# kfirc1503/generative-audio

Hardware: AMD Instinct MI355X
Metric: spectrogram-frames/sec, NPPC K=5 FullSubNet+ train step (higher is better)
Workload: dtype bf16

## Files before the change

### generative-audio_amd/csrc/train_ops.hip

```cpp
#include "common.h"
#include "nppc_hip.h"

namespace {

template <typename T>
__global__ __launch_bounds__(256) void transpose_kernel(const T* __restrict__ in, T* __restrict__ out, int rows, int cols,
                                                        long ld_in, long ld_out, long sIn, long sOut, int relu) {
  __shared__ float tile[32][33];
  in += (size_t)blockIdx.z * sIn;
  out += (size_t)blockIdx.z * sOut;
  const int r0 = blockIdx.x * 32, c0 = blockIdx.y * 32;
  const int tx = threadIdx.x & 31, ty = threadIdx.x >> 5;
  for (int i = ty; i < 32; i += 8) {
    const int r = r0 + i, c = c0 + tx;
    float v = 0.f;
    if (r < rows && c < cols) v = to_f32<T>(in[(size_t)r * ld_in + c]);
    if (relu) v = fmaxf(v, 0.f);
    tile[i][tx] = v;
  }
  __syncthreads();
  for (int i = ty; i < 32; i += 8) {
    const int c = c0 + i, r = r0 + tx;
    if (c < cols && r < rows) out[(size_t)c * ld_out + r] = from_f32<T>(tile[tx][i]);
  }
// ... 308 lines not shown
  for (long e = (long)blockIdx.x * blockDim.x + threadIdx.x; e < total; e += (long)gridDim.x * blockDim.x) {
    const int r = (int)(e / ncols), c = (int)(e % ncols);
    float s = 0.f;
    for (int k = 0; k < S; ++k) s += slabs[(size_t)k * slab_stride + (size_t)r * ld + col0 + c];
    int rr = r;
    if (permH > 0) {
      const int u = r >> 2, gp = r & 3;
      const int tg = gp == 0 ? 0 : (gp == 1 ? 2 : (gp == 2 ? 1 : 3));
      rr = tg * permH + u;
    }
    float* d = dst + (size_t)rr * dst_ld + c;
    *d = accumulate ? *d + s : s;
  }
}

__global__ void reduce_slabs_t_kernel(const float* __restrict__ slabs, int S, long slab_stride, long ld, float* __restrict__ dst,
                                      long dst_ld, int rows, int ncols, long sSlab, long sDst) {
  slabs += (size_t)blockIdx.z * sSlab;
  dst += (size_t)blockIdx.z * sDst;
  __shared__ float tile[32][33];
  const int c0 = blockIdx.x * 32, r0 = blockIdx.y * 32;
  const int tx = threadIdx.x & 31, ty = threadIdx.x >> 5;
  for (int i = ty; i < 32; i += 8) {
    const int c = c0 + i, r = r0 + tx;
    float a = 0.f;
    if (c < ncols && r < rows)
      for (int s = 0; s < S; ++s) a += slabs[(size_t)s * slab_stride + (size_t)c * ld + r];
    tile[i][tx] = a;
  }
  __syncthreads();
  for (int i = ty; i < 32; i += 8) {
    const int r = r0 + i, c = c0 + tx;
    if (r < rows && c < ncols) dst[(size_t)r * dst_ld + c] = tile[tx][i];
  }
}

__global__ void adam_kernel(float* __restrict__ p, const float* __restrict__ g, float* __restrict__ m, float* __restrict__ v,
                            long n, float lr, float b1, float b2, float eps, float wd, float bc1, float bc2_sqrt,
                            float gscale, const double* __restrict__ sumsq, float max_norm,
                            const unsigned* const* __restrict__ guards = nullptr, int n_guards = 0, float* poison = nullptr) {
  for (int i = 0; i < n_guards; ++i)
    if (*guards[i] != 0u) {
      if (poison && blockIdx.x == 0 && threadIdx.x == 0) *poison = __builtin_nanf("");
      return;
    }
  if (sumsq) {
    const float total = (float)sqrt(sumsq[0]) * gscale;
    const float coef = max_norm / (total + 1e-6f);
    gscale *= coef < 1.f ? coef : 1.f;
  }
  for (long i = (long)blockIdx.x * blockDim.x + threadIdx.x; i < n; i += (long)gridDim.x * blockDim.x) {
    float gi = g[i] * gscale;
    const float pi = p[i];
    if (wd != 0.f) gi += wd * pi;
    const float mi = b1 * m[i] + (1.f - b1) * gi;
    const float vi = b2 * v[i] + (1.f - b2) * gi * gi;
    m[i] = mi;
    v[i] = vi;
    const float denom = sqrtf(vi) / bc2_sqrt + eps;
    p[i] = pi - (lr / bc1) * (mi / denom);
  }
}

}

extern "C" {
// ... 147 lines not shown
  const double Nn = (double)F * (2 * nb + 4) * Tv;
  dim3 grid(Tv, B);
  hipStream_t s = (hipStream_t)stream;
  if (prec == NPPC_PREC_BF16)
    hipLaunchKernelGGL(sb_unfold_bwd_kernel<bf16_t>, grid, dim3(256), sm, s, (const bf16_t*)dx, scale, D, mult, (bf16_t*)dX0,
                       ldX, B, F, Tp, nb, Geff, Fo, KX, Nseq, Nn);
  else
    hipLaunchKernelGGL(sb_unfold_bwd_kernel<float>, grid, dim3(256), sm, s, (const float*)dx, scale, D, mult, (float*)dX0, ldX,
                       B, F, Tp, nb, Geff, Fo, KX, Nseq, Nn);
  NPPC_CHECK_LAUNCH();
  return NPPC_OK;
}

int nppc_reduce_slabs(const float* slabs, int S, long slab_stride, long ld, float* dst, long dst_ld, int rows, int col0,
                      int ncols, int permH, int accumulate, long sSlab, long sDst, int batch, void* stream) {
  if (!slabs || !dst || S < 1 || rows <= 0 || ncols <= 0) return NPPC_EBADARG;
  const long total = (long)rows * ncols;
  const int gx = (int)((total + 255) / 256 > 1024 ? 1024 : (total + 255) / 256);
  hipLaunchKernelGGL(reduce_slabs_kernel, dim3(gx, 1, batch), dim3(256), 0, (hipStream_t)stream, slabs, S, slab_stride, ld,
                     dst, dst_ld, rows, col0, ncols, permH, accumulate, sSlab, sDst);
  NPPC_CHECK_LAUNCH();
  return NPPC_OK;
}

int nppc_reduce_slabs_t(const float* slabs, int S, long slab_stride, long ld, float* dst, long dst_ld, int rows, int ncols,
                        long sSlab, long sDst, int batch, void* stream) {
  if (!slabs || !dst || S < 1 || rows <= 0 || ncols <= 0 || batch < 1) return NPPC_EBADARG;
  hipLaunchKernelGGL(reduce_slabs_t_kernel, dim3(ceil_div(ncols, 32), ceil_div(rows, 32), batch), dim3(256), 0,
                     (hipStream_t)stream, slabs, S, slab_stride, ld, dst, dst_ld, rows, ncols, sSlab, sDst);
  NPPC_CHECK_LAUNCH();
  return NPPC_OK;
}

int nppc_adam_step(float* p, const float* g, float* m, float* v, long n, double lr, double b1, double b2, double eps,
                   double wd, int step, double gscale, void* stream) {
  if (!p || !g || !m || !v || n <= 0 || step < 1) return NPPC_EBADARG;
  const double bc1 = 1.0 - pow(b1, (double)step);
  const double bc2s = sqrt(1.0 - pow(b2, (double)step));
  const int grid = (int)((n + 255) / 256 > 2048 ? 2048 : (n + 255) / 256);
  hipLaunchKernelGGL(adam_kernel, dim3(grid), dim3(256), 0, (hipStream_t)stream, p, g, m, v, n, (float)lr, (float)b1, (float)b2,
                     (float)eps, (float)wd, (float)bc1, (float)bc2s, (float)gscale, (const double*)nullptr, 0.f);
  NPPC_CHECK_LAUNCH();
  return NPPC_OK;
}

int nppc_adam_step_guarded(float* p, const float* g, float* m, float* v, long n, double lr, double b1, double b2, double eps,
                           double wd, int step, double gscale, const void* guards, int n_guards, float* poison, void* stream) {
  if (!p || !g || !m || !v || n <= 0 || step < 1 || n_guards < 0 || (n_guards > 0 && !guards)) return NPPC_EBADARG;
  const double bc1 = 1.0 - pow(b1, (double)step);
  const double bc2s = sqrt(1.0 - pow(b2, (double)step));
  const int grid = (int)((n + 255) / 256 > 2048 ? 2048 : (n + 255) / 256);
  hipLaunchKernelGGL(adam_kernel, dim3(grid), dim3(256), 0, (hipStream_t)stream, p, g, m, v, n, (float)lr, (float)b1, (float)b2,
                     (float)eps, (float)wd, (float)bc1, (float)bc2s, (float)gscale, (const double*)nullptr, 0.f,
                     (const unsigned* const*)guards, n_guards, poison);
  NPPC_CHECK_LAUNCH();
  return NPPC_OK;
}

int nppc_adam_step_clip(float* p, const float* g, float* m, float* v, long n, double lr, double b1, double b2, double eps,
                        double wd, int step, double gscale, const double* sumsq, double max_norm, void* stream) {
  if (!p || !g || !m || !v || !sumsq || n <= 0 || step < 1 || !(max_norm > 0)) return NPPC_EBADARG;
  const double bc1 = 1.0 - pow(b1, (double)step);
  const double bc2s = sqrt(1.0 - pow(b2, (double)step));
  const int grid = (int)((n + 255) / 256 > 2048 ? 2048 : (n + 255) / 256);
  hipLaunchKernelGGL(adam_kernel, dim3(grid), dim3(256), 0, (hipStream_t)stream, p, g, m, v, n, (float)lr, (float)b1, (float)b2,
                     (float)eps, (float)wd, (float)bc1, (float)bc2s, (float)gscale, sumsq, (float)max_norm);
// ... 6 lines not shown
```

### generative-audio_amd/nppc_audio/_hip.py

```python
import ctypes
import os

import torch

_HERE = os.path.dirname(os.path.abspath(__file__))
LIB_PATH = os.environ.get("NPPC_HIP_LIB") or os.path.join(_HERE, "libnppc_hip.so")

PREC_BF16 = 0
PREC_F32 = 1
_ERR = {1: "bad argument", 2: "kernel launch failed", 3: "unsupported shape/configuration"}

_lib = None

c_p = ctypes.c_void_p
c_i = ctypes.c_int
c_l = ctypes.c_long
c_f = ctypes.c_float


def lib():
    global _lib
    if _lib is None:
        if not os.path.exists(LIB_PATH):
            raise RuntimeError(
# ... 108 lines not shown
                         I, I, I, I, I, F, L, L, L, I, I, P],
    "nppc_tcn_mid_bwd_finish": [P, L, P, L, I, I, I, P, P, P, P, P, P, P, P, P, P, I, I, L, L, I, I, P],
    "nppc_gemm_nt_colsum": [I, I, P, L, L, P, L, L, P, L, L, P, L, P, L, L, I, I, I, I, I, I, I, P, P],
    "nppc_gemm_nt_gn": [I, P, L, L, P, L, L, P, L, L, P, P, L, P, L, L, P, L, D, F, I, I, I, I, I, I, I, P],
    "nppc_tcn_pack_sconv": [I, P, P, P, P, P, P, P, I, I, I, I, I, I, L, L, L, L, P],
    "nppc_gemm_nt_splitk": [I, P, L, P, L, P, L, I, I, L, I, P],
    "nppc_gemm_tn_splitk": [P, L, P, L, P, L, I, I, L, I, P],
    "nppc_gemm_tn_splitk_rowsum": [P, L, P, L, P, L, I, I, L, I, P, P],
    "nppc_gemm_tn_splitk2": [P, L, P, L, I, P, L, I, P, L, I, L, I, P, P],
    "nppc_gemm_tn_splitk_batched": [P, L, L, P, L, L, P, L, L, I, I, L, I, I, P],
    "nppc_reduce_slabs_t": [P, I, L, L, P, L, I, I, L, L, I, P],
    "nppc_gemm_tn_splitk_taps": [P, L, P, L, P, L, I, I, L, I, I, I, P],
    "nppc_tcn_dwconv": [I, P, P, P, P, P, P, P, P, P, I, I, I, I, I, I, F, L, L, L, I, P],
    "nppc_tcn_gn_apply": [I, P, P, P, P, P, I, I, I, I, I, F, L, L, L, I, P],
    "nppc_pack_matrix": [I, P, P, I, I, I, I, I, P],
    "nppc_pack_matrix_batched": [I, P, P, I, I, I, I, I, I, I, L, L, L, L, P],
    "nppc_subband_mean": [I, P, I, P, I, L, P, P, P, I, I, I, I, I, P],
    "nppc_subband_stage": [I, P, I, P, I, L, P, P, I, I, I, I, I, I, I, I, P],
    "nppc_sb_head": [I, P, P, P, P, L, I, I, I, I, I, P],
    "nppc_gram": [P, P, P, P, P, I, I, L, P],
    "nppc_combine": [P, P, P, P, P, P, P, I, I, L, P],
    "nppc_gs_solve": [P, P, P, I, I, I, P],
    "nppc_gs_bwd_solve": [P, P, P, P, I, I, I, P],
    "nppc_loss_solve": [P, P, P, P, P, P, P, P, P, P, I, I, P],
    "nppc_loss_bwd_coef": [P, P, P, F, F, P, I, I, P],
    "nppc_loss_bwd_coef_dev": [P, P, P, P, F, F, P, I, I, P],
    "nppc_transpose": [I, P, P, I, I, L, L, L, L, I, I, P],
    "nppc_colsum": [I, P, P, I, I, L, L, L, I, P, L, P],
    "nppc_colsum_scratch_elems": [I, I, I, PL],
    "nppc_sb_head_bwd": [I, P, P, P, P, P, P, L, I, I, I, I, I, P],
    "nppc_subband_stage_bwd": [I, P, P, P, P, P, P, I, I, I, I, I, L, I, I, I, P],
    "nppc_subband_unfold_bwd": [I, P, P, P, P, P, I, I, I, I, I, I, I, I, P],
    "nppc_reduce_slabs": [P, I, L, L, P, L, I, I, I, I, I, L, L, I, P],
    "nppc_adam_step": [P, P, P, P, L, D, D, D, D, D, I, D, P],
    "nppc_adam_step_guarded": [P, P, P, P, L, D, D, D, D, D, I, D, P, I, P, P],
    "nppc_loss_solve_eps": [P, P, P, P, P, P, P, P, P, P, I, I, D, I, P],
    "nppc_loss_solve_obj": [P, P, P, P, P, P, P, P, P, P, I, I, D, I, F, P, P],
    "nppc_mix_snr": [P, P, P, F, P, P, P, I, I, P],
    "nppc_inpaint_prepare": [P, P, P, I, F, P, P, P, I, I, I, I, I, P],
    "nppc_time_to_spec_mask": [P, P, I, I, I, I, I, I, P],
    "nppc_stft_pair": [P, P, P, P, I, I, I, I, P],
    "nppc_dropout": [I, P, L, L, I, F, L, I, P, P],
    "nppc_pca_work_elems": [I, I, I, PL],
    "nppc_pca_batch": [P, I, I, I, I, P, P, P, P, P, P, P],
    "nppc_pair_loss": [P, P, P, P, P, P, P, P, P, I, I, L, D, P],
    "nppc_pair_loss_bwd": [P, P, P, P, F, F, P, I, I, L, P],
    "nppc_metric_rows": [P, P, P, P, P, L, P],
    "nppc_rows_gram": [P, I, P, I, L, P, P],
    "nppc_sumsq": [P, L, P, P],
    "nppc_adam_step_clip": [P, P, P, P, L, D, D, D, D, D, I, D, P, D, P],
    "nppc_logmag": [P, P, L, I, L, P, P],
    "nppc_standardize": [P, P, L, I, L, P, P, P],
    "nppc_unet_stage_map": [I, P, L, P, L, I, I, I, I, P],
    "nppc_conv_pack": [I, P, P, P, I, I, I, I, I, I, I, P],
    "nppc_conv_fwd": [I, P, L, P, P, L, P, P, P, F, I, I, I, I, I, I, I, P],
    "nppc_conv_fwd_stats": [I, P, L, P, P, L, P, I, I, I, I, I, I, I, P, P],
    "nppc_bn_stats_from_parts": [P, I, I, I, I, I, P, P, P],
    "nppc_conv_wgrad": [I, P, L, P, L, P, I, I, I, I, I, I, I, P],
    "nppc_conv_thin_part_elems": [PL],
    "nppc_conv3x3_thin_fwd": [I, P, L, P, P, P, P, F, P, L, I, I, I, I, I, P],
    "nppc_conv3x3_thin_wgrad": [I, P, L, P, L, P, P, I, I, I, I, I, P],
    "nppc_conv1x1_thin_fwd": [I, P, L, P, P, P, L, I, I, I, I, I, P],
    "nppc_conv1x1_thin_bwd_data": [I, P, L, P, P, L, I, I, I, I, I, P],
    "nppc_conv1x1_thin_wgrad": [I, P, L, P, L, P, P, I, I, I, I, I, P],
    "nppc_conv_wgrad_transposed": [I, I],
    "nppc_conv_wgrad_reduce": [I, P, I, I, I, P, I, I, I, P],
# ... 74 lines not shown
    "nppc_flac_decode_host": [P, L, P, L, P, L, P],
    "nppc_flac_work_elems": [L, PL],
    "nppc_flac_scan": [P, L, P, I, P, L, P],
    "nppc_flac_parse": [P, P, I, P, L, P],
    "nppc_flac_chain": [P, P, I, P, L, P, P],
    "nppc_flac_decode": [P, P, I, P, L, P, L, P, L, P],
    "nppc_flac_stream_md5": [P, L, P, P, P],
    "nppc_flac_md5_host": [P, L, I, I, P],
    "nppc_flac_md5": [P, L, P, I, P, P, P, P, P, P],
    "nppc_resample_sinc_shape": [I, I, I, I, I, PI, PL, PL, PL, PI],
    "nppc_resample_sinc": [P, L, P, I, P, I, I, I, I, I, P, L, P],
}
_bound = set()
PROFILE = None


def call(name, *args):
    fn = getattr(lib(), name)
    if name not in _bound:
        fn.argtypes = SIGS[name]
        fn.restype = c_i
        _bound.add(name)
    conv = [ptr(a) if (isinstance(a, torch.Tensor) or a is None) else a for a in args]
    if PROFILE is None:
        check(fn(*conv), name)
        return
    e0, e1 = torch.cuda.Event(enable_timing=True), torch.cuda.Event(enable_timing=True)
    e0.record()
    check(fn(*conv), name)
    e1.record()
    PROFILE.append((name, e0, e1))


def colsum(prec, M, out, rows, cols, ld, sM, sOut, batch, scratch_for, s):
    n = ctypes.c_long()
    call("nppc_colsum_scratch_elems", rows, cols, batch, ctypes.byref(n))
    sc = scratch_for(n.value)
    call("nppc_colsum", prec, M, out, rows, cols, ld, sM, sOut, batch, sc, sc.numel(), s)
```

### generative-audio_amd/nppc_audio/engine.py

```python
import ctypes
import os

import numpy as np
import torch

from . import _hip as H
from .ops_lstm import (PackedLSTM, PackedLSTMBwd, ROW_PAD, WGRAD_SPLITS, bwd_head_fusable, forward_x_ld, lstm2_backward, lstm2_forward,
                       own_workspaces, padded_rows,
                       rows_view, workspace)

TCN_HIDDEN = 512
TCN_DILATIONS = (1, 2, 5, 9, 1, 2, 5, 9)
BRANCHES = ("", "_real", "_imag")
EPI_PLAIN, EPI_PRELU_STATS, EPI_RESIDUAL, EPI_RELU, EPI_PLAIN_F32, EPI_MASK_POS = 0, 1, 2, 3, 4, 5


def rup(a, b):
    return (a + b - 1) // b * b


TCN_WGRAD_ON_SIDE = os.environ.get("NPPC_TCN_WGRAD_SIDE", "1") != "0"
TCN_WGRAD_SPLITS = int(os.environ.get("NPPC_TCN_S2", "8"))
FC_WGRAD_AT_END = os.environ.get("NPPC_FC_AT_END", "1") != "0"
TCN_WGRAD_MAIN_BLOCKS = int(os.environ.get("NPPC_TCN_WGRAD_MAIN_BLOCKS", "1"))
MID_FINISH_DEFER = os.environ.get("NPPC_MID_FINISH_DEFER", "1") != "0"
COLSUM_IN_GEMM = os.environ.get("NPPC_COLSUM_IN_GEMM", "1") != "0"
TN_PAIRED = os.environ.get("NPPC_TN_PAIRED", "1") != "0"
FUSED_HEAD = int(os.environ.get("NPPC_FUSED_HEAD", "3"))


class FlatParams:

    def __init__(self, module, device):
        named = list(module.named_parameters())
        total = sum(p.numel() for _, p in named)
        self.flat = torch.empty(total, dtype=torch.float32, device=device)
        self.grad = None
        self.off = {}
        o = 0
        for n, p in named:
            k = p.numel()
            self.flat[o:o + k].copy_(p.detach().reshape(-1))
            p.data = self.flat[o:o + k].view(p.shape)
            self.off[n] = (o, tuple(p.shape))
            o += k
        self.named = named

    def view(self, name):
        o, shp = self.off[name]
        return self.flat[o:o + int(np.prod(shp))].view(shp)

    def gview(self, name):
        o, shp = self.off[name]
        return self.grad[o:o + int(np.prod(shp))].view(shp)

    def version(self):
        return (self.flat._version, sum(p._version for _, p in self.named))

    def ensure_grad(self):
        if self.grad is None:
# ... 336 lines not shown
        q = "sb_model.sequence_model."
        Rr = Tv * Nseq
        ws = lambda name, shape, dtype=dt, zero=False: workspace(("eng", id(self), name), shape, dtype, dev, zero)
        jobs = [
            (dg1, 0, x_rows, KX, ("ih", q + "weight_ih_l0", q + "bias_ih_l0", q + "bias_hh_l0")),
            (dg2, 0, x_rows, KX, ("bias", None, q + "bias_ih_l1", q + "bias_hh_l1")),
            (dg2, 0, h1_rows, Hd, ("w", q + "weight_ih_l1")),
        ]
        if Tv > 1:
            jobs += [(dg1, Nseq, h1_rows, Hd, ("w", q + "weight_hh_l0")), (dg2, Nseq, h2_rows, Hd, ("w", q + "weight_hh_l1"))]

        def scatter(slab, S, rows, ncolsN, dest):
            kind = dest[0]
            if kind in ("ih", "w"):
                ncol = I if kind == "ih" else Hd
                H.call("nppc_reduce_slabs", slab, S, rows * ncolsN, ncolsN, self.g(dest[1]), ncol, K4, 0, ncol, Hd, 0, 0, 0, 1, s)
            if kind in ("ih", "bias"):
                H.call("nppc_reduce_slabs", slab, S, rows * ncolsN, ncolsN, self.g(dest[2]), 1, K4, I, 1, Hd, 0, 0, 0, 1, s)
                self.g(dest[3]).copy_(self.g(dest[2]))

        if self.prec == H.PREC_BF16 and K4 % 128 == 0 and Hd % 64 == 0 and KX % 64 == 0:
            S = WGRAD_SPLITS
            assert 64 * S <= ROW_PAD
            slab = ws("slab", (S * K4 * max(Hd, KX),), torch.float32)
            fold_bias = K4 % 256 == 0 and Hd % 128 == 0 and (K4 // 256) * (Hd // 128) * S >= 256
            if (guards is not None and TN_PAIRED and fold_bias and Hd % 192 == 0 and KX == 64 and Tv > 1
                    and (K4 // 256) * (Hd // 192 + 1) * S >= 256):
                h1_guard, h2_guard = guards
                rows = (Rr + 64 * S - 1) // (64 * S) * (64 * S)
                slab = ws("slab2", (S * K4 * 2 * Hd,), torch.float32)
                rsum = ws("rowsum", (S, K4), torch.float32)
                H.call("nppc_gemm_tn_splitk2", dg1, K4, h1_guard, Hd, Hd, x_rows, KX, KX, slab, Hd + KX, K4, rows, S, None, s)
                n1 = K4 * (Hd + KX)
                H.call("nppc_reduce_slabs", slab, S, n1, Hd + KX, self.g(q + "weight_hh_l0"), Hd, K4, 0, Hd, Hd, 0, 0, 0, 1, s)
                H.call("nppc_reduce_slabs", slab, S, n1, Hd + KX, self.g(q + "weight_ih_l0"), I, K4, Hd, I, Hd, 0, 0, 0, 1, s)
                H.call("nppc_reduce_slabs", slab, S, n1, Hd + KX, self.g(q + "bias_ih_l0"), 1, K4, Hd + I, 1, Hd, 0, 0, 0, 1, s)
                self.g(q + "bias_hh_l0").copy_(self.g(q + "bias_ih_l0"))
                H.call("nppc_gemm_tn_splitk2", dg2, K4, h1_rows, Hd, Hd, h2_guard, Hd, Hd, slab, 2 * Hd, K4, rows, S, rsum, s)
                n2 = K4 * 2 * Hd
                H.call("nppc_reduce_slabs", slab, S, n2, 2 * Hd, self.g(q + "weight_ih_l1"), Hd, K4, 0, Hd, Hd, 0, 0, 0, 1, s)
                H.call("nppc_reduce_slabs", slab, S, n2, 2 * Hd, self.g(q + "weight_hh_l1"), Hd, K4, Hd, Hd, Hd, 0, 0, 0, 1, s)
                H.call("nppc_reduce_slabs", rsum, S, K4, 1, self.g(q + "bias_ih_l1"), 1, K4, 0, 1, Hd, 0, 0, 0, 1, s)
                self.g(q + "bias_hh_l1").copy_(self.g(q + "bias_ih_l1"))
                jobs = []
            for dg, off, inp, width, dest in jobs:
                rows = (Rr - off + 64 * S - 1) // (64 * S) * (64 * S)
                if fold_bias and dest[0] == "bias":
                    continue
                if fold_bias and dest == ("w", q + "weight_ih_l1"):
                    rsum = ws("rowsum", (S, K4), torch.float32)
                    H.call("nppc_gemm_tn_splitk_rowsum", dg.view(-1)[off * K4:], K4, inp, width, slab, width, K4, width, rows, S,
                           rsum, s)
                    H.call("nppc_reduce_slabs", rsum, S, K4, 1, self.g(q + "bias_ih_l1"), 1, K4, 0, 1, Hd, 0, 0, 0, 1, s)
                    self.g(q + "bias_hh_l1").copy_(self.g(q + "bias_ih_l1"))
                else:
                    H.call("nppc_gemm_tn_splitk", dg.view(-1)[off * K4:], K4, inp, width, slab, width, K4, width, rows, S, s)
                scatter(slab, S, K4, width, dest)
            if head is not None:
                dyt_rows, O = head
                rows = (Rr + 64 * S - 1) // (64 * S) * (64 * S)
                H.call("nppc_gemm_tn_splitk", h2_rows, Hd, dyt_rows, 16, slab, 64, Hd, 64, rows, S, s)
                H.call("nppc_reduce_slabs_t", slab, S, Hd * 64, 64, self.g("sb_model.fc_output_layer.weight"), Hd, O, Hd, 0, 0, 1, s)
                H.colsum(self.prec, dyt_rows, self.g("sb_model.fc_output_layer.bias"), Rr, O, 16, 0, 0, 1,
                         lambda n: ws("cs_head", (n,), torch.float32), s)
            return
        bk = 64 if self.prec == H.PREC_BF16 else 32
        Sg = max(1, min(64, Rr // (16 * bk)))
        Rp = rup(Rr, bk * Sg)
        K4p, Hp, KXp = rup(K4, 128), rup(Hd, 128), rup(KX, 128)
        dgT = [ws("dg1T", (K4p, Rp), zero=True), ws("dg2T", (K4p, Rp), zero=True)]
        for src, dst in ((dg1, dgT[0]), (dg2, dgT[1])):
            H.call("nppc_transpose", self.prec, src, dst, Rr, K4, K4, Rp, 0, 0, 0, 1, s)
        slab = ws("slab", (Sg * K4p * max(Hp, KXp),), torch.float32)
        for dg, off, inp, width, dest in jobs:
            wp = rup(width, 128)
            name = f"inT_{id(inp)}_{off}"
# ... 94 lines not shown
            dXL = [ws(f"dX_{i}", (3, B, Tp, ldC)) for i in range(9)]
            a2L = [ws(f"a2_{i}", (3, B, Tp, TCN_HIDDEN), zero=True) for i in range(8)]
            h2L = [ws(f"h2b_{i}", (3, B, Tp, TCN_HIDDEN)) for i in range(8)]
            dXa, dXb = dXL[8], dXL[7]
        else:
            dXa = ws("dXa", (3, B, Tp, ldC))
            dXb = ws("dXb", (3, B, Tp, ldC))

        bk = 64 if prec == H.PREC_BF16 else 32
        cs_ok = tn_ok and COLSUM_IN_GEMM and ldF % bk == 0 and TCN_HIDDEN % bk == 0
        cp_all = ws("colpart", (8, 3, R // 128, ldC), torch.float32) if cs_ok else None
        cpL = [cp_all[i] for i in range(8)] if cs_ok else None
        if cs_ok:
            H.call("nppc_gemm_nt_colsum", prec, EPI_MASK_POS, dpre_fb, ldF, R * ldF, self.WfcT, ldF, ldC * ldF, dXa, ldC, R * ldC,
                   None, 0, X8, ldC, R * ldC, R, ldC, ldF, Tp, Tv, C, 3, cpL[7], s)
        else:
            H.call("nppc_gemm_nt", prec, EPI_MASK_POS, dpre_fb, ldF, R * ldF, self.WfcT, ldF, ldC * ldF, dXa, ldC, R * ldC, None, 0,
                   X8, ldC, R * ldC, None, 0, None, 0, R, ldC, ldF, Tp, Tv, C, 0, 3, 1, s)
        sAct = B * Tp * TCN_HIDDEN
        h1b = ws("h1b", (3, B, Tp, TCN_HIDDEN))
        h2b = ws("h2b", (3, B, Tp, TCN_HIDDEN))
        Smid = ws("Smid", (3, B, TCN_HIDDEN // 64, 8), torch.float64)
        n_part = H.mid_bwd_part_elems(B, TCN_HIDDEN, Tp, 3)
        Pmid = ws("Pmid", (8, n_part), torch.float32)
        lay = self.fp.off["fb_model.sequence_model.1.conv1x1.weight"][0] - self.fp.off["fb_model.sequence_model.0.conv1x1.weight"][0]

        def finish_mid(lo, hi):
            pre_ = f"fb_model.sequence_model.{lo}."
            H.call("nppc_tcn_mid_bwd_finish", Pmid[lo], n_part, cpL[lo] if cs_ok else None, 3 * (R // 128) * ldC, R // 128, ldC, C,
                   self.g(pre_ + "norm2.weight"), self.g(pre_ + "norm2.bias"), self.g(pre_ + "norm1.weight"), self.g(pre_ + "norm1.bias"),
                   self.g(pre_ + "depthwise_conv.weight"), self.g(pre_ + "depthwise_conv.bias"), self.g(pre_ + "prelu1.weight"),
                   self.g(pre_ + "prelu2.weight"), self.g(pre_ + "conv1x1.bias"), self.g(pre_ + "sconv.bias") if cs_ok else None,
                   B, TCN_HIDDEN, sP, lay, 3, hi - lo, s)
        early = self.grad_range_hook is not None and self.early_buckets_ok
        defer_finish = MID_FINISH_DEFER
        dXo, dXi = dXa, dXb
        for i in range(7, -1, -1):
            pre = f"fb_model.sequence_model.{i}."
            dil = TCN_DILATIONS[i]
            st1, st2 = d["stats"][i, 0], d["stats"][i, 1]
            y1, y2, Xin = d["y1"][i], d["y2"][i], d["X"][i]
            if tn_ok:
                dXo, dXi, a2, h2b = dXL[i + 1], dXL[i], a2L[i], h2L[i]
            else:
                a2 = d["a2"]
            if not cs_ok:
                H.colsum(prec, dXo, self.g(pre + "sconv.bias"), R, C, ldC, R * ldC, sP, 3,
                         lambda n: ws("cs_sconv", (n,), torch.float32), s)
            H.call("nppc_gemm_nt", prec, EPI_PLAIN, dXo, ldC, R * ldC, self.W2T[i], ldC, TCN_HIDDEN * ldC, h1b, TCN_HIDDEN,
                   sAct, None, 0, None, 0, 0, None, 0, None, 0, R, TCN_HIDDEN, ldC, Tp, Tv, TCN_HIDDEN, 0, 3, 1, s)
            H.call("nppc_tcn_mid_bwd", prec, h1b, y2, y1, st1, st2, Smid, Pmid[i], self.p(pre + "norm1.weight"), self.p(pre + "norm1.bias"),
                   self.p(pre + "norm2.weight"), self.p(pre + "norm2.bias"), self.p(pre + "depthwise_conv.weight"),
                   self.p(pre + "prelu1.weight"), self.p(pre + "prelu2.weight"), a2, h2b, self.g(pre + "norm2.weight"),
                   self.g(pre + "norm2.bias"), self.g(pre + "norm1.weight"), self.g(pre + "norm1.bias"),
                   self.g(pre + "depthwise_conv.weight"), self.g(pre + "depthwise_conv.bias"), self.g(pre + "prelu1.weight"),
                   self.g(pre + "prelu2.weight"), self.g(pre + "conv1x1.bias"),
                   cpL[i] if cs_ok else None, R // 128, ldC, C, self.g(pre + "sconv.bias") if cs_ok else None,
                   B, TCN_HIDDEN, Tp, Tv, dil, 1e-8, sAct, B * 2, sP, 3, 0 if defer_finish else 1, s)
            if i == 4 and early and defer_finish:
                finish_mid(4, 8)
            if tn_ok:
                inline = i < TCN_WGRAD_MAIN_BLOCKS
                wslab = ws("slab_main", (3 * S2 * TCN_HIDDEN * ldC,), torch.float32) if inline else slab2

                def sconv_wgrad(a2=a2, dXo=dXo, dest=self.g(pre + "sconv.weight"), wslab=wslab):
                    q = H.stream()
                    H.call("nppc_gemm_tn_splitk_batched", a2, TCN_HIDDEN, sAct, dXo, ldC, R * ldC, wslab, ldC,
                           S2 * TCN_HIDDEN * ldC, TCN_HIDDEN, ldC, R, S2, 3, q)
                    H.call("nppc_reduce_slabs_t", wslab, S2, TCN_HIDDEN * ldC, ldC, dest, TCN_HIDDEN, C, TCN_HIDDEN,
                           S2 * TCN_HIDDEN * ldC, sP, 3, q)
                if inline:
                    sconv_wgrad()
                else:
                    on_side(sconv_wgrad)
            else:
                H.call("nppc_transpose", prec, dXo, tA, R, ldC, ldC, R, R * ldC, sTA, 0, 3, s)
                H.call("nppc_transpose", prec, a2, tB, R, TCN_HIDDEN, TCN_HIDDEN, R, sAct, sTB, 0, 3, s)
                self._wgrad(tA, R, sTA, tB, R, sTB, Cr, TCN_HIDDEN, R, S2, pre + "sconv.weight", TCN_HIDDEN, C, TCN_HIDDEN,
                            slab2, batch=3, sDst=sP)
            if tn_ok:
                def c1_wgrad(h2b=h2b, Xin=Xin, dest=self.g(pre + "conv1x1.weight"), wslab=wslab):
                    q = H.stream()
                    H.call("nppc_gemm_tn_splitk_batched", h2b, TCN_HIDDEN, sAct, Xin, ldC, R * ldC, wslab, ldC,
                           S2 * TCN_HIDDEN * ldC, TCN_HIDDEN, ldC, R, S2, 3, q)
                    H.call("nppc_reduce_slabs", wslab, S2, TCN_HIDDEN * ldC, ldC, dest, C, TCN_HIDDEN, 0, C, 0, 0,
                           S2 * TCN_HIDDEN * ldC, sP, 3, q)
                if inline:
                    c1_wgrad()
                else:
                    on_side(c1_wgrad)
            else:
                H.call("nppc_transpose", prec, h2b, tA, R, TCN_HIDDEN, TCN_HIDDEN, R, sAct, sTA, 0, 3, s)
                H.call("nppc_transpose", prec, Xin, tB, R, ldC, ldC, R, R * ldC, sTB, 0, 3, s)
                self._wgrad(tA, R, sTA, tB, R, sTB, TCN_HIDDEN, ldC, R, S2, pre + "conv1x1.weight", C, TCN_HIDDEN, C, slab2,
                            batch=3, sDst=sP)
            if cs_ok and i > 0:
                H.call("nppc_gemm_nt_colsum", prec, EPI_RESIDUAL, h2b, TCN_HIDDEN, sAct, self.W1T[i], TCN_HIDDEN, ldC * TCN_HIDDEN,
                       dXi, ldC, R * ldC, None, 0, dXo, ldC, R * ldC, R, ldC, TCN_HIDDEN, Tp, Tv, C, 3, cpL[i - 1], s)
            else:
                H.call("nppc_gemm_nt", prec, EPI_RESIDUAL, h2b, TCN_HIDDEN, sAct, self.W1T[i], TCN_HIDDEN, ldC * TCN_HIDDEN, dXi, ldC,
                       R * ldC, None, 0, dXo, ldC, R * ldC, None, 0, None, 0, R, ldC, TCN_HIDDEN, Tp, Tv, C, 0, 3, 1, s)
            dXo, dXi = dXi, dXo
            if i == 4 and self.grad_range_hook is not None and self.early_buckets_ok:
                def blocks_done():
                    for br in BRANCHES:
                        a = self.fp.off[f"fb_model{br}.sequence_model.4.conv1x1.weight"][0]
                        b, shp = self.fp.off[f"fb_model{br}.sequence_model.7.sconv.bias"]
                        self.grad_range_hook(G, a, b + int(np.prod(shp)))
                on_side(blocks_done)
        if defer_finish:
            finish_mid(0, 4 if early else 8)
        if tn_ok:
            dXo = dXL[0]
        if self.nm == 1:
            H.call("nppc_subband_unfold_bwd", prec, dx, d["sbscale"], Dsb, self.mult, dXo[0], ldC, B, F, Tp, Tv, self.nb, self.G,
                   self.KX, s)
        sv = d["tsse_saved"]
        n_ws = ctypes.c_long()
        H.call("nppc_tsse_bwd_ws_elems", 3 * self.nm, B, F, self.ks[0], self.ks[1], self.ks[2], ctypes.byref(n_ws))
        dsg = ws("dsg", (n_ws.value,), torch.float32)
        att = "channel_attention."
        H.call("nppc_tsse_bwd_maps", prec, dXo, R * ldC, H.ptr_array(d["maps"]), 3 * self.nm, d["rs"],
               self.p(att + "smallConv1d.0.weight"), self.p(att + "middleConv1d.0.weight"), self.p(att + "largeConv1d.0.weight"),
               self.ks[0], self.ks[1], self.ks[2], self.p(att + "feature_concate_fc.weight"), self.p(att + "fc1.weight"),
               self.p(att + "fc2.weight"), self.sAtt, sv["ns"], sv["pre"], sv["sq"], sv["h1"], sv["sg"], dsg,
               self.g(att + "smallConv1d.0.weight"), self.g(att + "smallConv1d.0.bias"),
               self.g(att + "middleConv1d.0.weight"), self.g(att + "middleConv1d.0.bias"),
               self.g(att + "largeConv1d.0.weight"), self.g(att + "largeConv1d.0.bias"),
               self.g(att + "feature_concate_fc.weight"), self.g(att + "feature_concate_fc.bias"),
               self.g(att + "fc1.weight"), self.g(att + "fc1.bias"), self.g(att + "fc2.weight"), self.g(att + "fc2.bias"),
               B, F, T, self.la, Tp, ldC, s)
        if fc_at_end:
            fc_wgrad(ws("slab_fc", (3 * S2 * Fr * ldC,), torch.float32))
        if self.defer_join:
            self.join_pending = True
            FSNEngine._unjoined[id(self)] = self
        else:
            torch.cuda.current_stream().wait_stream(self._side)
        return G

    def side_stream(self):
        return self._side

    def prepack_on_side(self):
# ... 19 lines not shown
```

### include/nppc_hip.h

```cpp
#ifndef NPPC_HIP_H
#define NPPC_HIP_H
#ifdef __cplusplus
extern "C" {
#endif

int nppc_stft(const float* wave, float* re, float* im, float* mag , int B, int L, int nfft, int hop,
              void* stream);
int nppc_dropband(const float* in, float* out, int B, int C, int F, int T, int G, void* stream);
int nppc_cirm_build_compress(const float* nr, const float* ni, const float* cr, const float* ci, float* out, int B, int F,
                             int T, int G, float eps, void* stream);
int nppc_cirm_decompress_apply_conj(const float* crm, const float* nr, const float* ni, float* dec ,
                                    float* emag, float* ere, float* eim, int B, int F, int T, void* stream);

int nppc_cirm_decompress_apply(const float* crm, const float* nr, const float* ni, float* dec , float* emag,
                               float* ere, float* eim, int B, int F, int T, void* stream);
int nppc_istft(const float* re, const float* im, float* out, int B, int T, int nfft, int hop, int L, void* stream);

int nppc_rowsum(const float* x, double* sums, long R, int T, void* stream);
int nppc_tsse_fwd_maps(int prec, const float* const* maps, int nmaps, double* rowsum, const float* cw0, const float* cb0,
                       const float* cw1, const float* cb1, const float* cw2, const float* cb2, int ks0, int ks1, int ks2,
                       const float* fcw, const float* fcb, const float* w1, const float* b1, const float* w2, const float* b2, long sW,
                       float* scale, float* ns, float* pre, float* sq, float* h1, float* sg, void* X0, long sY, int B, int C, int T,
                       int look_ahead, int Tp, int ld, void* stream);
int nppc_tsse_bwd_ws_elems(int nmaps, int B, int C, int ks0, int ks1, int ks2, long* elems);
// ... 48 lines not shown
                        const float* wd, void* dz, float* dwd, float* dbd, int B, int Cc, int Tp, int Tv, int dil, float eps,
                        long sAct, long sSt, long sP, int batch, void* stream);
int nppc_tcn_mid_bwd_part_elems(int B, int Cc, int Tp, int batch, long* n);
int nppc_tcn_mid_bwd(int prec, const void* dA, const void* y2, const void* y1, const double* st1, const double* st2, double* S,
                     float* part,
                     const float* gamma1, const float* beta1, const float* gamma2, const float* beta2, const float* wd,
                     const float* slope1, const float* slope2, void* a2, void* dpre1, float* dgamma2, float* dbeta2,
                     float* dgamma1, float* dbeta1, float* dwd, float* dbd, float* dslope1, float* dslope2, float* dbias1,
                     const float* colpart, int cp_tiles, int cp_ld, int cp_cols, float* dbias2, int B,
                     int Cc, int Tp, int Tv, int dil, float eps, long sAct, long sSt, long sP, int batch, int finish_now,
                     void* stream);
int nppc_tcn_mid_bwd_finish(const float* part, long partL, const float* colpart, long colpartL, int cp_tiles, int cp_ld,
                            int cp_cols, float* dgamma2, float* dbeta2, float* dgamma1, float* dbeta1, float* dwd, float* dbd,
                            float* dslope1, float* dslope2, float* dbias1, float* dbias2, int B, int Cc, long sP, long sL,
                            int batch, int nblk, void* stream);
int nppc_gemm_nt_gn(int prec, const void* A, long lda, long sA, const void* Wg, long ldb, long sB, void* C, long ldc, long sC,
                    const float* u, const float* v, long sUV, const void* res, long ldres, long sRes, const double* stats,
                    long sStats, double cnt, float eps, int R, int N, int K, int Tp, int Tv, int Nv, int batch, void* stream);
int nppc_gemm_nt_colsum(int prec, int epi, const void* A, long lda, long sA, const void* B, long ldb, long sB, void* C, long ldc,
                        long sC, const float* bias, long sBias, const void* res, long ldres, long sRes, int R, int N, int K,
                        int Tp, int Tv, int Nv, int batch, float* colpart, void* stream);
int nppc_tcn_pack_sconv(int prec, const float* W, const float* gamma, const float* beta, const float* bias, void* Wg, float* u,
                        float* v, int N, int K, int Npad, int ldd, int n_a, int n_b, long src_stride_a, long src_stride_b,
                        long dst_stride_a, long dst_stride_b, void* stream);
int nppc_transpose(int prec, const void* in, void* out, int rows, int cols, long ld_in, long ld_out, long sIn, long sOut,
                   int relu, int batch, void* stream);
int nppc_colsum_scratch_elems(int rows, int cols, int batch, long* n);
int nppc_colsum(int prec, const void* M, float* out, int rows, int cols, long ld, long sM, long sOut, int batch,
                float* scratch, long scratch_elems, void* stream);
int nppc_reduce_slabs_t(const float* slabs, int S, long slab_stride, long ld, float* dst, long dst_ld, int rows, int ncols,
                        long sSlab, long sDst, int batch, void* stream);
int nppc_reduce_slabs(const float* slabs, int S, long slab_stride, long ld, float* dst, long dst_ld, int rows, int col0,
                      int ncols, int permH, int accumulate, long sSlab, long sDst, int batch, void* stream);

int nppc_subband_mean(int prec, const void* src, int ldS, const void* fb, int ldF, long strideFb, const float* mult,
                      float* scale, double* work, int B, int F, int Tp, int Tv, int nfeat, void* stream);
int nppc_subband_stage(int prec, const void* src, int ldS, const void* fb, int ldF, long strideFb, const float* scale,
                       void* x, int B, int F, int Tp, int Tv, int nb, int G, int KX, int ones_col, void* stream);
int nppc_subband_stage_bwd(int prec, const void* dx, const void* x, const void* fb, const float* scale, double* D,
                           void* dpre, int B, int F, int Tp, int Tv, int ldF, long strideFb, int nb, int G, int KX,
                           void* stream);
int nppc_subband_unfold_bwd(int prec, const void* dx, const float* scale, const double* D, const float* mult, void* dX0,
                            int ldX, int B, int F, int Tp, int Tv, int nb, int G, int KX, void* stream);
int nppc_sb_head(int prec, const void* h2, const void* wh, const float* bias, float* out, long Nseq, int Tn, int la,
                 int Hd, int O, int Fo, void* stream);
int nppc_sb_head_bwd(int prec, const float* dout, const void* whT, const void* h2, void* dh2, float* dWh, float* dbh,
                     long Nseq, int Tn, int la, int Hd, int O, int Fo, void* stream);

int nppc_lstm2_packed_elems(int I, int H, long* n1, long* n2, int* kx);
int nppc_lstm2_pack_weights(int prec, const float* w_ih0, const float* w_hh0, const float* b_ih0, const float* b_hh0,
                            const float* w_ih1, const float* w_hh1, const float* b_ih1, const float* b_hh1, int I, int H,
                            void* wp1, void* wp2, float* bias1, float* bias2, void* stream);
int nppc_lstm2_fwd(int prec, int train, int mtile, const void* x, const void* wp1, const void* wp2, const float* bias1,
                   const float* bias2, void* h2, void* h1, void* g1, void* g2, void* c1, void* c2, long N, int Tn, int I,
                   int H, void* stream);
int nppc_lstm2_coop_plan(int prec, int train, long N, int H, int n_cu, int* G, int* mtile, int* clusters);
int nppc_lstm2_fwd_coop(int prec, int train, int G, int mtile, const void* x, const void* wp1, const void* wp2,
                        const float* bias1, const float* bias2, void* h2, void* h1, void* g1, void* g2, void* c1, void* c2,
                        void* xch, long xch_bytes, unsigned* flags, long N, int Tn, int I, int H, void* stream);
int nppc_lstm2_fwd_coop_head(int prec, int train, int mtile, const void* x, const void* wp1, const void* wp2,
                             const float* bias1, const float* bias2, void* h2, void* h1, void* g1, void* g2, void* c1, void* c2,
                             void* xch, long xch_bytes, unsigned* flags, long N, int Tn, int I, int H, const void* whp,
                             float* hpart, int O, int x_ld , void* stream);
int nppc_sb_head_finalize(const float* hpart, int G, const float* bias, float* out, long Nseq, int Tn, int la, int O, int Fo,
                          void* stream);
int nppc_lstm2_ws_plan(int prec, long N, int H, int I, int n_cu, int* clusters, int* nch_max);
// ... 324 lines not shown
```

Measured before the change: 255,000.

## Fuse LSTM and TCN split-K weight-gradient slab reductions into batched finish kernels

Adds two kernels that reduce split-K weight-gradient slabs with vectorized nontemporal loads. The LSTM one writes weight_hh, weight_ih and both bias copies in a single launch instead of three reductions plus a copy. The TCN one defers the sconv and conv1x1 reductions across all blocks into per-layer persistent slab buffers and finishes them in one batched launch, partly on a side stream. This cuts launch count and small-kernel overhead in exchange for a larger slab workspace and a fallback path when shapes or alignment are unsupported.

Result: no change. 254,100 (-0.3%).

```diff
diff --git a/generative-audio_amd/csrc/train_ops.hip b/generative-audio_amd/csrc/train_ops.hip
--- a/generative-audio_amd/csrc/train_ops.hip
+++ b/generative-audio_amd/csrc/train_ops.hip
@@ -364,6 +364,111 @@
   for (int i = ty; i < 32; i += 8) {
     const int r = r0 + i, c = c0 + tx;
     if (r < rows && c < ncols) dst[(size_t)r * dst_ld + c] = tile[tx][i];
+  }
+}
+
+__device__ __forceinline__ f32x4 slab_sum4(const float* __restrict__ p, int S, long slab_stride, int n) {
+  f32x4 acc = {0.f, 0.f, 0.f, 0.f};
+  if (n >= 4) {
+    int k = 0;
+    for (; k + 8 <= S; k += 8) {
+      u32x4 v[8];
+#pragma unroll
+      for (int j = 0; j < 8; ++j) v[j] = ld_nt16(p + (size_t)(k + j) * slab_stride);
+#pragma unroll
+      for (int j = 0; j < 8; ++j) acc = acc + __builtin_bit_cast(f32x4, v[j]);
+    }
+    for (; k < S; ++k) acc = acc + __builtin_bit_cast(f32x4, ld_nt16(p + (size_t)k * slab_stride));
+  } else {
+    for (int k = 0; k < S; ++k)
+      for (int j = 0; j < n; ++j) acc[j] = acc[j] + __builtin_nontemporal_load(p + (size_t)k * slab_stride + j);
+  }
+  return acc;
+}
+
+__global__ void __launch_bounds__(256)
+lstm_wgrad_finish_kernel(const float* __restrict__ slabs, const float* __restrict__ rowsum, int S, long slab_stride, long ld, int H,
+                         int wB, float* __restrict__ dA, float* __restrict__ dB, float* __restrict__ b0, float* __restrict__ b1,
+                         int cpr, int nb_main, int vec) {
+  const int rows = 4 * H;
+  if ((int)blockIdx.x >= nb_main) {
+    const int r = ((int)blockIdx.x - nb_main) * 256 + threadIdx.x;
+    if (r >= rows) return;
+    float acc = 0.f;
+    for (int k = 0; k < S; ++k) acc = acc + rowsum[(size_t)k * rows + r];
+    const int gp = r & 3, rr = (gp == 0 ? 0 : (gp == 1 ? 2 : (gp == 2 ? 1 : 3))) * H + (r >> 2);
+    b0[rr] = acc;
+    b1[rr] = acc;
+    return;
+  }
+  const long e = (long)blockIdx.x * 256 + threadIdx.x;
+  if (e >= (long)rows * cpr) return;
+  const int r = (int)(e / cpr), c0 = 4 * (int)(e % cpr);
+  const int nread = H + wB + (rowsum ? 0 : 1);
+  const int n = nread - c0 < 4 ? nread - c0 : 4;
+  const f32x4 acc = slab_sum4(slabs + (size_t)r * ld + c0, S, slab_stride, n);
+  const int gp = r & 3, rr = (gp == 0 ? 0 : (gp == 1 ? 2 : (gp == 2 ? 1 : 3))) * H + (r >> 2);
+  if (c0 < H) {
+    float* d = dA + (size_t)rr * H + c0;
+    if (vec & 1) *reinterpret_cast<f32x4*>(d) = acc;
+    else { d[0] = acc[0]; d[1] = acc[1]; d[2] = acc[2]; d[3] = acc[3]; }
+  } else if (n == 4 && c0 + 4 <= H + wB && (vec & 2)) {
+    *reinterpret_cast<f32x4*>(dB + (size_t)rr * wB + (c0 - H)) = acc;
+  } else {
+    for (int j = 0; j < n; ++j) {
+      const int c = c0 + j - H;
+      if (c < wB) dB[(size_t)rr * wB + c] = acc[j];
+      else { b0[rr] = acc[j]; b1[rr] = acc[j]; }
+    }
+  }
+}
+
+__global__ void __launch_bounds__(256)
+tcn_wgrad_finish_kernel(const float* __restrict__ slabs, long sBlk, long sProd, long sBr, int S, long slab_stride, int Hc, int C,
+                        long ldC, float* __restrict__ d0, float* __restrict__ d1, long sP, long lay, int tilesC, int vec) {
+  __shared__ float tile[64][33];
+  const int prod = blockIdx.y & 1, br = blockIdx.y >> 1;
+  slabs += (size_t)blockIdx.z * sBlk + (size_t)prod * sProd + (size_t)br * sBr;
+  const int cT = (int)blockIdx.x % tilesC, kT = (int)blockIdx.x / tilesC;
+  const int ch = threadIdx.x & 15, kr = threadIdx.x >> 4;
+  const int c0 = cT * 64 + 4 * ch;
+  const int n = C - c0 < 4 ? C - c0 : 4;
+  f32x4 acc[2];
+#pragma unroll
+  for (int h = 0; h < 2; ++h) {
+    const int k = kT * 32 + kr + 16 * h;
+    acc[h] = f32x4{0.f, 0.f, 0.f, 0.f};
+    if (k < Hc && n > 0) acc[h] = slab_sum4(slabs + (size_t)k * ldC + c0, S, slab_stride, n);
+  }
+  if (prod == 1) {
+    float* d = d1 + (size_t)blockIdx.z * lay + (size_t)br * sP;
+#pragma unroll
+    for (int h = 0; h < 2; ++h) {
+      const int k = kT * 32 + kr + 16 * h;
+      if (k >= Hc || n <= 0) continue;
+      float* q = d + (size_t)k * C + c0;
+      if (n == 4 && (vec & 2)) *reinterpret_cast<f32x4*>(q) = acc[h];
+      else
+        for (int j = 0; j < n; ++j) q[j] = acc[h][j];
+    }
+    return;
+  }
+#pragma unroll
+  for (int h = 0; h < 2; ++h)
+#pragma unroll
+    for (int j = 0; j < 4; ++j) tile[4 * ch + j][kr + 16 * h] = acc[h][j];
+  __syncthreads();
+  float* d = d0 + (size_t)blockIdx.z * lay + (size_t)br * sP;
+  const int c = cT * 64 + (threadIdx.x >> 2), k0 = kT * 32 + 4 * (threadIdx.x & 3);
+#pragma unroll
+  for (int h = 0; h < 2; ++h) {
+    const int k = k0 + 16 * h, kl = 4 * (threadIdx.x & 3) + 16 * h;
+    if (c >= C || k >= Hc) continue;
+    const float* t = tile[threadIdx.x >> 2] + kl;
+    float* q = d + (size_t)c * Hc + k;
+    if (k + 4 <= Hc && (vec & 1)) *reinterpret_cast<f32x4*>(q) = f32x4{t[0], t[1], t[2], t[3]};
+    else
+      for (int j = 0; j < 4 && k + j < Hc; ++j) q[j] = t[j];
   }
 }
 
@@ -577,6 +682,41 @@
   return NPPC_OK;
 }
 
+static inline bool al16(const void* p) { return ((uintptr_t)p) % 16 == 0; }
+
+int nppc_lstm_wgrad_finish(const float* slabs, const float* rowsum, int S, long slab_stride, long ld, int H, int wB, float* dA,
+                           float* dB, float* b0, float* b1, void* stream) {
+  if (!slabs || !dA || !dB || !b0 || !b1 || S < 1 || H < 1 || wB < 1 || ld < 1 || slab_stride < 4L * H * ld) return NPPC_EBADARG;
+  const int nread = H + wB + (rowsum ? 0 : 1);
+  if (nread > ld) return NPPC_EBADARG;
+  if (H % 4 || ld % 4 || slab_stride % 4 || !al16(slabs)) return NPPC_EUNSUPPORTED;
+  const int cpr = ceil_div(nread, 4);
+  const long nb_main = ((long)4 * H * cpr + 255) / 256;
+  const long nb = nb_main + (rowsum ? ceil_div(4 * H, 256) : 0);
+  if (nb > 0x7fffffffL) return NPPC_EUNSUPPORTED;
+  const int vec = (al16(dA) ? 1 : 0) | (al16(dB) && wB % 4 == 0 ? 2 : 0);
+  hipLaunchKernelGGL(lstm_wgrad_finish_kernel, dim3((unsigned)nb), dim3(256), 0, (hipStream_t)stream, slabs, rowsum, S,
+                     slab_stride, ld, H, wB, dA, dB, b0, b1, cpr, (int)nb_main, vec);
+  NPPC_CHECK_LAUNCH();
+  return NPPC_OK;
+}
+
+int nppc_tcn_wgrad_finish(const float* slabs, long sBlk, long sProd, long sBr, int S, long slab_stride, int Hc, int C, long ldC,
+                          float* d_sconv, float* d_c1, long sP, long lay, int batch, int nblk, void* stream) {
+  if (!slabs || !d_sconv || !d_c1 || S < 1 || Hc < 1 || C < 1 || ldC < C || slab_stride < (long)Hc * ldC || batch < 1 || nblk < 1)
+    return NPPC_EBADARG;
+  if (ldC % 4 || slab_stride % 4 || sBlk % 4 || sProd % 4 || sBr % 4 || !al16(slabs)) return NPPC_EUNSUPPORTED;
+  const int tilesC = ceil_div(C, 64);
+  const long nbx = (long)tilesC * ceil_div(Hc, 32);
+  if (nbx > 0x7fffffffL || 2L * batch > 65535 || nblk > 65535) return NPPC_EUNSUPPORTED;
+  const bool strides4 = sP % 4 == 0 && lay % 4 == 0;
+  const int vec = (al16(d_sconv) && Hc % 4 == 0 && strides4 ? 1 : 0) | (al16(d_c1) && C % 4 == 0 && strides4 ? 2 : 0);
+  hipLaunchKernelGGL(tcn_wgrad_finish_kernel, dim3((unsigned)nbx, 2 * batch, nblk), dim3(256), 0, (hipStream_t)stream, slabs, sBlk,
+                     sProd, sBr, S, slab_stride, Hc, C, ldC, d_sconv, d_c1, sP, lay, tilesC, vec);
+  NPPC_CHECK_LAUNCH();
+  return NPPC_OK;
+}
+
 int nppc_adam_step(float* p, const float* g, float* m, float* v, long n, double lr, double b1, double b2, double eps,
                    double wd, int step, double gscale, void* stream) {
   if (!p || !g || !m || !v || n <= 0 || step < 1) return NPPC_EBADARG;
diff --git a/generative-audio_amd/nppc_audio/_hip.py b/generative-audio_amd/nppc_audio/_hip.py
--- a/generative-audio_amd/nppc_audio/_hip.py
+++ b/generative-audio_amd/nppc_audio/_hip.py
@@ -164,6 +164,8 @@
     "nppc_subband_stage_bwd": [I, P, P, P, P, P, P, I, I, I, I, I, L, I, I, I, P],
     "nppc_subband_unfold_bwd": [I, P, P, P, P, P, I, I, I, I, I, I, I, I, P],
     "nppc_reduce_slabs": [P, I, L, L, P, L, I, I, I, I, I, L, L, I, P],
+    "nppc_lstm_wgrad_finish": [P, P, I, L, L, I, I, P, P, P, P, P],
+    "nppc_tcn_wgrad_finish": [P, L, L, L, I, L, I, I, L, P, P, L, L, I, I, P],
     "nppc_adam_step": [P, P, P, P, L, D, D, D, D, D, I, D, P],
     "nppc_adam_step_guarded": [P, P, P, P, L, D, D, D, D, D, I, D, P, I, P, P],
     "nppc_loss_solve_eps": [P, P, P, P, P, P, P, P, P, P, I, I, D, I, P],
@@ -304,6 +306,16 @@
     PROFILE.append((name, e0, e1))
 
 
+def call_supported(name, *args):
+    try:
+        call(name, *args)
+    except RuntimeError as e:
+        if str(e) != f"{name} failed: {_ERR[3]}":
+            raise
+        return False
+    return True
+
+
 def colsum(prec, M, out, rows, cols, ld, sM, sOut, batch, scratch_for, s):
     n = ctypes.c_long()
     call("nppc_colsum_scratch_elems", rows, cols, batch, ctypes.byref(n))
diff --git a/generative-audio_amd/nppc_audio/engine.py b/generative-audio_amd/nppc_audio/engine.py
--- a/generative-audio_amd/nppc_audio/engine.py
+++ b/generative-audio_amd/nppc_audio/engine.py
@@ -26,6 +26,7 @@
 MID_FINISH_DEFER = os.environ.get("NPPC_MID_FINISH_DEFER", "1") != "0"
 COLSUM_IN_GEMM = os.environ.get("NPPC_COLSUM_IN_GEMM", "1") != "0"
 TN_PAIRED = os.environ.get("NPPC_TN_PAIRED", "1") != "0"
+WGRAD_FINISH = os.environ.get("NPPC_WGRAD_FINISH", "1") != "0"
 FUSED_HEAD = int(os.environ.get("NPPC_FUSED_HEAD", "3"))
 
 
@@ -428,16 +429,22 @@
                 rsum = ws("rowsum", (S, K4), torch.float32)
                 H.call("nppc_gemm_tn_splitk2", dg1, K4, h1_guard, Hd, Hd, x_rows, KX, KX, slab, Hd + KX, K4, rows, S, None, s)
                 n1 = K4 * (Hd + KX)
-                H.call("nppc_reduce_slabs", slab, S, n1, Hd + KX, self.g(q + "weight_hh_l0"), Hd, K4, 0, Hd, Hd, 0, 0, 0, 1, s)
-                H.call("nppc_reduce_slabs", slab, S, n1, Hd + KX, self.g(q + "weight_ih_l0"), I, K4, Hd, I, Hd, 0, 0, 0, 1, s)
-                H.call("nppc_reduce_slabs", slab, S, n1, Hd + KX, self.g(q + "bias_ih_l0"), 1, K4, Hd + I, 1, Hd, 0, 0, 0, 1, s)
-                self.g(q + "bias_hh_l0").copy_(self.g(q + "bias_ih_l0"))
+                if not (WGRAD_FINISH and H.call_supported(
+                        "nppc_lstm_wgrad_finish", slab, None, S, n1, Hd + KX, Hd, I, self.g(q + "weight_hh_l0"),
+                        self.g(q + "weight_ih_l0"), self.g(q + "bias_ih_l0"), self.g(q + "bias_hh_l0"), s)):
+                    H.call("nppc_reduce_slabs", slab, S, n1, Hd + KX, self.g(q + "weight_hh_l0"), Hd, K4, 0, Hd, Hd, 0, 0, 0, 1, s)
+                    H.call("nppc_reduce_slabs", slab, S, n1, Hd + KX, self.g(q + "weight_ih_l0"), I, K4, Hd, I, Hd, 0, 0, 0, 1, s)
+                    H.call("nppc_reduce_slabs", slab, S, n1, Hd + KX, self.g(q + "bias_ih_l0"), 1, K4, Hd + I, 1, Hd, 0, 0, 0, 1, s)
+                    self.g(q + "bias_hh_l0").copy_(self.g(q + "bias_ih_l0"))
                 H.call("nppc_gemm_tn_splitk2", dg2, K4, h1_rows, Hd, Hd, h2_guard, Hd, Hd, slab, 2 * Hd, K4, rows, S, rsum, s)
                 n2 = K4 * 2 * Hd
-                H.call("nppc_reduce_slabs", slab, S, n2, 2 * Hd, self.g(q + "weight_ih_l1"), Hd, K4, 0, Hd, Hd, 0, 0, 0, 1, s)
-                H.call("nppc_reduce_slabs", slab, S, n2, 2 * Hd, self.g(q + "weight_hh_l1"), Hd, K4, Hd, Hd, Hd, 0, 0, 0, 1, s)
-                H.call("nppc_reduce_slabs", rsum, S, K4, 1, self.g(q + "bias_ih_l1"), 1, K4, 0, 1, Hd, 0, 0, 0, 1, s)
-                self.g(q + "bias_hh_l1").copy_(self.g(q + "bias_ih_l1"))
+                if not (WGRAD_FINISH and H.call_supported(
+                        "nppc_lstm_wgrad_finish", slab, rsum, S, n2, 2 * Hd, Hd, Hd, self.g(q + "weight_ih_l1"),
+                        self.g(q + "weight_hh_l1"), self.g(q + "bias_ih_l1"), self.g(q + "bias_hh_l1"), s)):
+                    H.call("nppc_reduce_slabs", slab, S, n2, 2 * Hd, self.g(q + "weight_ih_l1"), Hd, K4, 0, Hd, Hd, 0, 0, 0, 1, s)
+                    H.call("nppc_reduce_slabs", slab, S, n2, 2 * Hd, self.g(q + "weight_hh_l1"), Hd, K4, Hd, Hd, Hd, 0, 0, 0, 1, s)
+                    H.call("nppc_reduce_slabs", rsum, S, K4, 1, self.g(q + "bias_ih_l1"), 1, K4, 0, 1, Hd, 0, 0, 0, 1, s)
+                    self.g(q + "bias_hh_l1").copy_(self.g(q + "bias_ih_l1"))
                 jobs = []
             for dg, off, inp, width, dest in jobs:
                 rows = (Rr - off + 64 * S - 1) // (64 * S) * (64 * S)
@@ -598,6 +605,33 @@
                    self.g(pre_ + "depthwise_conv.weight"), self.g(pre_ + "depthwise_conv.bias"), self.g(pre_ + "prelu1.weight"),
                    self.g(pre_ + "prelu2.weight"), self.g(pre_ + "conv1x1.bias"), self.g(pre_ + "sconv.bias") if cs_ok else None,
                    B, TCN_HIDDEN, sP, lay, 3, hi - lo, s)
+        n_ws = 3 * S2 * TCN_HIDDEN * ldC
+        wfin = tn_ok and WGRAD_FINISH
+        Wsl = ws("wslabs", (8, 2, n_ws), torch.float32) if wfin else None
+
+        def finish_w_on(lo, hi):
+            if hi <= lo:
+                return
+            q = H.stream()
+            pre_ = f"fb_model.sequence_model.{lo}."
+            if H.call_supported("nppc_tcn_wgrad_finish", Wsl[lo], 2 * n_ws, n_ws, S2 * TCN_HIDDEN * ldC, S2, TCN_HIDDEN * ldC,
+                                TCN_HIDDEN, C, ldC, self.g(pre_ + "sconv.weight"), self.g(pre_ + "conv1x1.weight"), sP, lay, 3,
+                                hi - lo, q):
+                return
+            for j in range(lo, hi):
+                pre_ = f"fb_model.sequence_model.{j}."
+                H.call("nppc_reduce_slabs_t", Wsl[j, 0], S2, TCN_HIDDEN * ldC, ldC, self.g(pre_ + "sconv.weight"), TCN_HIDDEN, C,
+                       TCN_HIDDEN, S2 * TCN_HIDDEN * ldC, sP, 3, q)
+                H.call("nppc_reduce_slabs", Wsl[j, 1], S2, TCN_HIDDEN * ldC, ldC, self.g(pre_ + "conv1x1.weight"), C, TCN_HIDDEN, 0, C,
+                       0, 0, S2 * TCN_HIDDEN * ldC, sP, 3, q)
+
+        def finish_w(lo, hi):
+            if not wfin:
+                return
+            mb = min(max(TCN_WGRAD_MAIN_BLOCKS, 0), 8)
+            finish_w_on(lo, min(hi, mb))
+            if max(lo, mb) < hi:
+                on_side(lambda: finish_w_on(max(lo, mb), hi))
         early = self.grad_range_hook is not None and self.early_buckets_ok
         defer_finish = MID_FINISH_DEFER
         dXo, dXi = dXa, dXb
@@ -627,10 +661,17 @@
                 finish_mid(4, 8)
             if tn_ok:
                 inline = i < TCN_WGRAD_MAIN_BLOCKS
-                wslab = ws("slab_main", (3 * S2 * TCN_HIDDEN * ldC,), torch.float32) if inline else slab2
-
-                def sconv_wgrad(a2=a2, dXo=dXo, dest=self.g(pre + "sconv.weight"), wslab=wslab):
+                if wfin:
+                    wslab = None
+                else:
+                    wslab = ws("slab_main", (3 * S2 * TCN_HIDDEN * ldC,), torch.float32) if inline else slab2
+
+                def sconv_wgrad(a2=a2, dXo=dXo, dest=self.g(pre + "sconv.weight"), wslab=wslab, i=i):
                     q = H.stream()
+                    if wfin:
+                        H.call("nppc_gemm_tn_splitk_batched", a2, TCN_HIDDEN, sAct, dXo, ldC, R * ldC, Wsl[i, 0], ldC,
+                               S2 * TCN_HIDDEN * ldC, TCN_HIDDEN, ldC, R, S2, 3, q)
+                        return
                     H.call("nppc_gemm_tn_splitk_batched", a2, TCN_HIDDEN, sAct, dXo, ldC, R * ldC, wslab, ldC,
                            S2 * TCN_HIDDEN * ldC, TCN_HIDDEN, ldC, R, S2, 3, q)
                     H.call("nppc_reduce_slabs_t", wslab, S2, TCN_HIDDEN * ldC, ldC, dest, TCN_HIDDEN, C, TCN_HIDDEN,
@@ -645,8 +686,12 @@
                 self._wgrad(tA, R, sTA, tB, R, sTB, Cr, TCN_HIDDEN, R, S2, pre + "sconv.weight", TCN_HIDDEN, C, TCN_HIDDEN,
                             slab2, batch=3, sDst=sP)
             if tn_ok:
-                def c1_wgrad(h2b=h2b, Xin=Xin, dest=self.g(pre + "conv1x1.weight"), wslab=wslab):
+                def c1_wgrad(h2b=h2b, Xin=Xin, dest=self.g(pre + "conv1x1.weight"), wslab=wslab, i=i):
                     q = H.stream()
+                    if wfin:
+                        H.call("nppc_gemm_tn_splitk_batched", h2b, TCN_HIDDEN, sAct, Xin, ldC, R * ldC, Wsl[i, 1], ldC,
+                               S2 * TCN_HIDDEN * ldC, TCN_HIDDEN, ldC, R, S2, 3, q)
+                        return
                     H.call("nppc_gemm_tn_splitk_batched", h2b, TCN_HIDDEN, sAct, Xin, ldC, R * ldC, wslab, ldC,
                            S2 * TCN_HIDDEN * ldC, TCN_HIDDEN, ldC, R, S2, 3, q)
                     H.call("nppc_reduce_slabs", wslab, S2, TCN_HIDDEN * ldC, ldC, dest, C, TCN_HIDDEN, 0, C, 0, 0,
@@ -668,6 +713,8 @@
                        R * ldC, None, 0, dXo, ldC, R * ldC, None, 0, None, 0, R, ldC, TCN_HIDDEN, Tp, Tv, C, 0, 3, 1, s)
             dXo, dXi = dXi, dXo
             if i == 4 and self.grad_range_hook is not None and self.early_buckets_ok:
+                finish_w(4, 8)
+
                 def blocks_done():
                     for br in BRANCHES:
                         a = self.fp.off[f"fb_model{br}.sequence_model.4.conv1x1.weight"][0]
@@ -676,6 +723,7 @@
                 on_side(blocks_done)
         if defer_finish:
             finish_mid(0, 4 if early else 8)
+        finish_w(0, 4 if early else 8)
         if tn_ok:
             dXo = dXL[0]
         if self.nm == 1:
diff --git a/include/nppc_hip.h b/include/nppc_hip.h
--- a/include/nppc_hip.h
+++ b/include/nppc_hip.h
@@ -104,6 +104,10 @@
                         long sSlab, long sDst, int batch, void* stream);
 int nppc_reduce_slabs(const float* slabs, int S, long slab_stride, long ld, float* dst, long dst_ld, int rows, int col0,
                       int ncols, int permH, int accumulate, long sSlab, long sDst, int batch, void* stream);
+int nppc_lstm_wgrad_finish(const float* slabs, const float* rowsum, int S, long slab_stride, long ld, int H, int wB, float* dA,
+                           float* dB, float* b0, float* b1, void* stream);
+int nppc_tcn_wgrad_finish(const float* slabs, long sBlk, long sProd, long sBr, int S, long slab_stride, int Hc, int C, long ldC,
+                          float* d_sconv, float* d_c1, long sP, long lay, int batch, int nblk, void* stream);
 
 int nppc_subband_mean(int prec, const void* src, int ldS, const void* fb, int ldF, long strideFb, const float* mult,
                       float* scale, double* work, int B, int F, int Tp, int Tv, int nfeat, void* stream);
```
